# reglab/aquaculture

Hardware: AMD Instinct MI355X
Metric: 640px tiles/sec (whole node) YOLOv5m bf16 (higher is better)
Workload: dtype bf16

## Files before the change

aquaculture_amd/csrc/conv1x1_direct.hip:

```cpp
#include "conv_device.h"

using namespace aqdev;

namespace {

struct C1Params {
    const char* in;
    char* out;
    const char* w;
    const float* bias;
    const char* zero;
    int in_ld_b, out_ld_b;
    int npix, n_tiles, act;
    float out_inv_scale;
};

constexpr int kNW = 12;

template <int KS, int MBT, int MBW, int NBW> struct C1Geom {
    static constexpr int CIN = 32 * KS, COUT = 16 * MBT, CB = CIN / 8;
    static constexpr int MG = MBT / MBW;
    static constexpr int PG = kNW / MG;
    static constexpr int TP = PG * NBW * 16;
    static constexpr int SPP = CB + 2;
    static constexpr int PXB = SPP * 16;
    static constexpr int NQ = (TP * SPP + 63) / 64;
    static constexpr int XPB = NQ * 1024;
    static constexpr int LDS = 2 * XPB + COUT * 4;
    static constexpr int NST = NBW;
    static_assert(MBT % MBW == 0 && kNW % MG == 0 && LDS <= 160 * 1024, "shape");
};

__device__ __forceinline__ f32x4 c1_silu4(f32x4 v) {
    const f32x4 t = v * -1.44269504f;
    f32x4 d = {__builtin_amdgcn_exp2f(t[0]), __builtin_amdgcn_exp2f(t[1]), __builtin_amdgcn_exp2f(t[2]), __builtin_amdgcn_exp2f(t[3])};
    d = d + 1.0f;
    const f32x4 r = {__builtin_amdgcn_rcpf(d[0]), __builtin_amdgcn_rcpf(d[1]), __builtin_amdgcn_rcpf(d[2]), __builtin_amdgcn_rcpf(d[3])};
    return v * r;
}

template <int KS, int MBT, int MBW, int NBW, bool F8OUT = false>
__global__ __launch_bounds__(kNW * 64) void conv1x1_direct_kernel(const C1Params p) {
    using G = C1Geom<KS, MBT, MBW, NBW>;
    extern __shared__ __attribute__((aligned(16))) char smem[];
    float* s_b = (float*)(smem + 2 * G::XPB);

    const int tid = threadIdx.x, lane = tid & 63;
    const int wave = __builtin_amdgcn_readfirstlane(tid >> 6);
    static_assert(MBW == 2, "the paired-row layout below is written for two M blocks per wave");
    const int mb0 = (wave % G::MG) * MBW, pg = wave / G::MG;
    const int g = lane >> 4, l15 = lane & 15;
    const int cbase = mb0 * 16 + g * 8;

    bf16x8 wv[KS][MBW];
#pragma unroll
    for (int s = 0; s < KS; ++s)
#pragma unroll
        for (int m = 0; m < MBW; ++m) wv[s][m] = ((const bf16x8*)p.w)[((size_t)(mb0 + m) * KS + s) * 64 + lane];
    for (int i = tid; i < G::COUT; i += kNW * 64) s_b[i] = p.bias[i];

    auto issue_dma = [&](int tile, char* xb) {
        const long long n0 = (long long)tile * G::TP;
#pragma unroll 1
        for (int q = wave; q < G::NQ; q += kNW) {
            const int slot = q * 64 + lane;
            const int px = slot / G::SPP, part = slot - px * G::SPP;
            const bool valid = px < G::TP && part < G::CB && n0 + px < p.npix;
            const char* src = p.in + (n0 + px) * p.in_ld_b + part * 16;
            glds16(valid ? src : p.zero, xb + q * 1024);
        }
    };

    int tile = first_tile(gridDim.x, blockIdx.x);
    if (tile < p.n_tiles) issue_dma(tile, smem);
    int cur = 0;
    bool prev_full = false;
    for (; tile < p.n_tiles; tile += gridDim.x, cur ^= 1) {
        const long long n0 = (long long)tile * G::TP;
        const char* s_x = smem + cur * G::XPB;
        if (prev_full) wait_vmcnt<G::NST>(); else wait_vmcnt<0>();
        asm volatile("s_waitcnt lgkmcnt(0)" ::: "memory");
        __builtin_amdgcn_s_barrier();
        asm volatile("" ::: "memory");
// ... 27 lines not shown
                    q0[e] = __builtin_amdgcn_fmed3f(q0[e], -448.0f, 448.0f);
                    q1[e] = __builtin_amdgcn_fmed3f(q1[e], -448.0f, 448.0f);
                }
                int w0 = __builtin_amdgcn_cvt_pk_fp8_f32(q0[0], q0[1], 0, false);
                w0 = __builtin_amdgcn_cvt_pk_fp8_f32(q0[2], q0[3], w0, true);
                int w1 = __builtin_amdgcn_cvt_pk_fp8_f32(q1[0], q1[1], 0, false);
                w1 = __builtin_amdgcn_cvt_pk_fp8_f32(q1[2], q1[3], w1, true);
                if (n0 + px < p.npix) *(uint2*)(p.out + (n0 + px) * p.out_ld_b + cbase) = make_uint2((unsigned)w0, (unsigned)w1);
            } else if (n0 + px < p.npix)
                *(uint4*)(p.out + (n0 + px) * p.out_ld_b + cbase * 2) =
                    make_uint4(pack_bf16x2(v0[0], v0[1]), pack_bf16x2(v0[2], v0[3]), pack_bf16x2(v1[0], v1[1]), pack_bf16x2(v1[2], v1[3]));
        }
    }
}

template <int KS, int MBT, int MBW, int NBW, bool F8OUT = false>
int launch_c1(C1Params p, hipStream_t stream) {
    using G = C1Geom<KS, MBT, MBW, NBW>;
    auto fn = conv1x1_direct_kernel<KS, MBT, MBW, NBW, F8OUT>;
    int cus = 0;
    AQ_CHECK_HIP(aq_kernel_lds((const void*)fn, G::LDS));
    AQ_CHECK_HIP(aq_cus(&cus));
    p.n_tiles = (p.npix + G::TP - 1) / G::TP;
    long long grid = cus;
    if (grid > p.n_tiles) grid = p.n_tiles;
    hipLaunchKernelGGL(fn, dim3((unsigned)grid), dim3(kNW * 64), G::LDS, stream, p);
    AQ_CHECK_HIP(hipGetLastError());
    return AQ_OK;
}

}

extern "C" int aq_conv1x1_direct_supported(int cin, int cout) {
    return (cin == 96 && cout == 96) || (cin == 192 && cout == 192) || (cin == 384 && (cout == 192 || cout == 384));
// ... 30 lines not shown
               "conv1x1_direct: channel slices must be 8-aligned and inside their rows");
    C1Params p{};
    p.in = (const char*)in_dev + (size_t)in_choff * 2; p.in_ld_b = in_ld * 2;
    p.out = (char*)out_dev + (size_t)out_choff * 2; p.out_ld_b = out_ld * 2;
    p.w = (const char*)packed_w_dev; p.bias = bias_dev;
    p.npix = (int)npix; p.act = act;
    p.zero = aq_zero_page();
    AQ_REQUIRE(p.zero, "conv1x1_direct: zero page allocation failed");
    const hipStream_t st = (hipStream_t)stream;
    if (cin == 96) return launch_c1<3, 6, 2, 4>(p, st);
    if (cin == 192) return launch_c1<6, 12, 2, 4>(p, st);
    if (cout == 192) return launch_c1<12, 12, 2, 2>(p, st);
    return launch_c1<12, 24, 2, 4>(p, st);
}


extern "C" int aq_conv1x1_direct_f8out(const void* in_dev, int in_ld, int in_choff, void* out_dev, int out_pitch_bytes, int out_byte_off, int cin,
                                       int cout, const void* packed_w_dev, const float* bias_dev, long long npix, int act, float out_scale,
                                       void* stream) {
    AQ_REQUIRE(in_dev && out_dev && packed_w_dev && bias_dev, "conv1x1_direct_f8out: null pointer");
    AQ_REQUIRE((cin == 192 && cout == 192) || (cin == 384 && cout == 384), "conv1x1_direct_f8out: unsupported %d -> %d", cin, cout);
    AQ_REQUIRE(npix > 0 && sg::conv1x1_direct_fits(npix) && out_scale > 0.0f, "conv1x1_direct_f8out: bad pixel count or scale");
    AQ_REQUIRE(in_ld % 8 == 0 && in_choff % 8 == 0 && in_choff + cin <= in_ld && out_pitch_bytes % 8 == 0 && out_byte_off % 8 == 0 &&
                   out_byte_off + cout <= out_pitch_bytes, "conv1x1_direct_f8out: slices must be 8-byte aligned and inside their rows");
    C1Params p{};
    p.in = (const char*)in_dev + (size_t)in_choff * 2; p.in_ld_b = in_ld * 2;
    p.out = (char*)out_dev + out_byte_off; p.out_ld_b = out_pitch_bytes;
    p.w = (const char*)packed_w_dev; p.bias = bias_dev;
    p.npix = (int)npix; p.act = act; p.out_inv_scale = 1.0f / out_scale;
    p.zero = aq_zero_page();
// ... 6 lines not shown
```

aquaculture_amd/csrc/engine.cpp:

```cpp
#include "aq_common.h"
#include <unistd.h>
#include <string>

#include <cstdarg>
#include <cstdio>
#include <cstdlib>
#include <cstring>
#include <string>
#include <atomic>
#include <dlfcn.h>
#include <vector>

namespace {
thread_local char g_err[512] = "";
}

void aq_set_error(const char* fmt, ...) {
    va_list ap;
    va_start(ap, fmt);
    vsnprintf(g_err, sizeof(g_err), fmt, ap);
    va_end(ap);
}

extern "C" const char* aq_last_error(void) { return g_err; }
// ... 123 lines not shown
}

struct aq_engine {
    int device = 0;
    aq_model_desc desc{};
    std::vector<aq_tensor_desc> tensors;
    std::vector<aq_op_desc> ops;
    std::vector<PackedW> packed;
    std::vector<int> conv_cfg;
    int nms_agnostic = 0;
    unsigned long long nms_cls_lo = ~0ULL, nms_cls_hi = ~0ULL;
    struct Tuned { int B = 0, H = 0, W = 0; std::vector<int> cfg; };
    std::vector<Tuned> tuned;
    int tuned_cur = -1;
    bool tuning = false;
    void* zero_page = nullptr;
    int lay_B = 0, lay_H = 0, lay_W = 0;
    bool lay_aug = false;
    int run_H = 0, run_W = 0;
    std::vector<TensorPlace> place;
    size_t off_pred = 0, off_cand = 0, off_cand_rows = 0, off_cand_count = 0, off_cand_wide = 0, off_nms = 0, off_taps = 0, total_bytes = 0;
    int N = 0;
    aq_augment_pass aug[3] = {};
    std::vector<int> aug_family[3], aug_cfg[3];
    void* last_ws = nullptr;
    const uint8_t* last_tiles = nullptr;
    float* calib_amax = nullptr;
    std::vector<int> last_family, last_cfg;
    bool prof = false;
    int ring = 0;
// ... 305 lines not shown
}

bool c3tail_active(aq_engine* e, int oi, int last, int B) {
    if (!e->packed[oi].w_tail || oi + 1 >= last || e->calib_amax || e->tuning) return false;
    const int ci = oi + 1;
    const PackedW& pc = e->packed[ci];
    if (pc.direct_cfg != AQ_CONV_CFG_DIRECT1X1 || (pc.f8_consumer >= 0 && f8_pair_active(e, pc.f8_consumer, B))) return false;
    const aq_engine::Tuned* tt = tuned_for(e);
    const int cfg = e->conv_cfg[ci] >= 0 ? e->conv_cfg[ci] : tt ? tt->cfg[ci] : -1;
    if (cfg != AQ_CONV_CFG_DIRECT1X1) return false;
    const aq_op_desc& b = e->ops[oi];
    const aq_op_desc& c = e->ops[ci];
    const TensorPlace& pl = e->place[b.src.tensor];
    return aq_bottleneck_c3tail_supported(B, pl.h, pl.w, e->tensors[b.src.tensor].channels, e->tensors[c.src.tensor].channels,
                                          e->tensors[c.dst.tensor].channels) != 0;
}

struct AugRun {
    int pass;
    const aq_augment_pass* ps;
    int H0, W0;
    const aq_tap* ytab;
    const aq_tap* xtab;
};

int run_plan(aq_engine* e, const uint8_t* tiles, int B, int H, int W, void* ws, size_t ws_bytes,
             float* pred_out, aq_det* dets, int32_t* counts, float conf, float iou, int max_det, hipStream_t stream,
             int first = 0, int last = -1, const AugRun* ar = nullptr) {
    AQ_REQUIRE(e && tiles && ws, "infer: null pointer");
    const int n_ops = (int)e->ops.size();
// ... 21 lines not shown
    int32_t* cand_count = (int32_t*)((char*)ws + e->off_cand_count);
    float* cand_rows = (float*)((char*)ws + e->off_cand_rows);
    const char* use_sd = getenv("AQ_STEMDOWN");
    const bool stemdown = use_sd && *use_sd == '1' && prec == AQ_BF16 && n_ops > 2 && e->ops[0].kind == AQ_OP_STEM && e->ops[1].kind == AQ_OP_DOWNBLOCK &&
                          e->ops[0].dst.channels == 48 && e->ops[1].src.tensor == e->ops[0].dst.tensor && e->ops[1].src.ch_off == e->ops[0].dst.ch_off &&
                          aq_stemdown_supported(H, W) && ((uintptr_t)tiles & 3) == 0 && !scaled;
    const bool fuse_heads = dets != nullptr && heads_fused(e);
    bool heads_started = ar != nullptr;
    int heads_done = 0;
    for (int oi = 0; oi < first; ++oi)
        if (fuse_heads && e->ops[oi].kind == AQ_OP_CONV && e->ops[oi].level >= 0) {
            heads_started = true;
            ++heads_done;
        }
    int tail_conv = -1;
    for (int oi = first; oi < last; ++oi) {
        const aq_op_desc& op = e->ops[oi];
        if (ev) AQ_CHECK_HIP(hipEventRecord(ev[oi], stream));
        const bool mark = g_roctx.on();
        if (mark) {
            char name[96];
            snprintf(name, sizeof name, "aq op %02d kind %d: %d -> %d ch, k%d s%d%s", oi, op.kind, op.src.channels, op.dst.channels, op.k, op.stride,
                     op.level >= 0 ? " (detect head)" : "");
            g_roctx.push(name);
        }
        switch (op.kind) {
        case AQ_OP_PREPROCESS:
            if (scaled)
                rc = aq_preprocess_s2d_scaled(tiles, ar->H0, ar->W0, ar->ytab, ar->xtab, ar->ps->h, ar->ps->w, tptr(e, ws, tiles, op.dst.tensor), B, H, W,
                                              prec, stream);
            else
                rc = aq_preprocess_s2d(tiles, tptr(e, ws, tiles, op.dst.tensor), B, H, W, prec, stream);
            break;
        case AQ_OP_CONV:
            if (oi == tail_conv) {
                note_launch(e, oi, AQ_FAM_DIRECT1X1, AQ_CONV_CFG_DIRECT1X1);
                break;
            }
            if (ar && op.level >= 0 && !((ar->ps->level_mask >> op.level) & 1)) {
                note_launch(e, oi, AQ_FAM_NONE);
                break;
            }
            if (fuse_heads && op.level >= 0) {
                int32_t* wide = (int32_t*)((char*)ws + e->off_cand_wide);
                if (!heads_started) {
                    AQ_CHECK_HIP(hipMemsetAsync(wide, 0, sizeof(int32_t) * B * kCountStride, stream));
                    heads_started = true;
                }
                const TensorPlace& pl = e->place[op.src.tensor];
                int off = 0;
                for (int l = 0; l < op.level; ++l) off += e->desc.na * (H / (int)e->desc.stride[l]) * (W / (int)e->desc.stride[l]);
// ... 61 lines not shown
                                 e->packed[0].w, e->packed[0].bias, e->packed[oi].w, e->packed[oi].bias, B, H, W, stream);
                break;
            }
            rc = aq_downblock(tptr(e, ws, tiles, op.src.tensor), e->tensors[op.src.tensor].channels, op.src.ch_off,
                              tptr(e, ws, tiles, op.dst.tensor), e->tensors[op.dst.tensor].channels, op.dst.ch_off,
                              e->packed[oi].w, e->packed[oi].bias, B, pl.h, pl.w, stream);
            break;
        }
        case AQ_OP_SPPF_POOL: {
            const TensorPlace& pl = e->place[op.src.tensor];
            rc = aq_sppf_pool(tptr(e, ws, tiles, op.src.tensor), e->tensors[op.src.tensor].channels, op.src.ch_off,
                              op.src.channels, B, pl.h, pl.w, prec, stream);
            break;
        }
        case AQ_OP_UPSAMPLE2X: {
            const TensorPlace& pl = e->place[op.src.tensor];
            rc = aq_upsample2x(tptr(e, ws, tiles, op.src.tensor), e->tensors[op.src.tensor].channels, op.src.ch_off,
                               tptr(e, ws, tiles, op.dst.tensor), e->tensors[op.dst.tensor].channels, op.dst.ch_off,
                               op.src.channels, B, pl.h, pl.w, prec, stream);
            break;
        }
        case AQ_OP_DECODE: {
            if (fuse_heads) break;
            const float* heads[3];
            for (int l = 0; l < 3; ++l) heads[l] = (const float*)tptr(e, ws, tiles, e->desc.head_tensor[l]);
            float anchors[3 * 8 * 2];
            for (int l = 0; l < 3; ++l)
                for (int a = 0; a < e->desc.na; ++a) {
                    anchors[(l * e->desc.na + a) * 2] = e->desc.anchors_px[l][a][0];
                    anchors[(l * e->desc.na + a) * 2 + 1] = e->desc.anchors_px[l][a][1];
// ... 199 lines not shown
    if (x3) compute_desc.precision = AQ_FP32;
    d = &compute_desc;
    e->desc = *d;
    e->tensors.assign(d->tensors, d->tensors + d->n_tensors);
    e->ops.assign(d->ops, d->ops + d->n_ops);
    e->desc.tensors = e->tensors.data();
    e->desc.ops = e->ops.data();
    e->packed.resize(e->ops.size());
    e->conv_cfg.assign(e->ops.size(), -1);
    const int eb = aq_elem_bytes(d->precision);
    auto fail = [&](int rc) { aq_engine_destroy(e); return rc; };
    if (hipMalloc(&e->zero_page, 4096) != hipSuccess || hipMemset(e->zero_page, 0, 4096) != hipSuccess) {
        aq_set_error("engine_create: zero page allocation failed");
        return fail(AQ_ERR_NOMEM);
    }
    const char* use_tail = getenv("AQ_C3TAIL");
    for (size_t oi = 0; d->precision == AQ_BF16 && !(use_tail && *use_tail == '0') && oi + 1 < e->ops.size(); ++oi) {
        const aq_op_desc& b = e->ops[oi];
        const aq_op_desc& c = e->ops[oi + 1];
        if (b.kind != AQ_OP_BOTTLENECK || c.kind != AQ_OP_CONV || !b.weight || !b.bias || !c.weight || !c.bias) continue;
        if (b.src.channels != 48 || b.dst.channels != 48 || b.k != 3 || b.dst.tensor < 0 || b.dst.tensor >= d->n_tensors || b.dst.ch_off != 0 ||
            e->tensors[b.dst.tensor].channels != 96 || b.src.tensor == b.dst.tensor)
            continue;
        if (c.k != 1 || c.stride != 1 || c.act != 1 || c.res.tensor >= 0 || c.level >= 0 || c.src.tensor != b.dst.tensor || c.src.ch_off != 0 ||
            c.src.channels != 96 || c.dst.channels != 96 || c.dst.tensor < 0 || c.dst.tensor >= d->n_tensors || c.dst.tensor == c.src.tensor ||
            c.dst.tensor == b.src.tensor || c.dst.ch_off % 8 || e->tensors[c.dst.tensor].channels % 8 || e->tensors[c.dst.tensor].dtype != AQ_T_ACT)
            continue;
        bool read_later = false;
        for (size_t oj = oi + 2; oj < e->ops.size(); ++oj)
            for (const aq_slice* s : {&e->ops[oj].src, &e->ops[oj].res})
// ... 551 lines not shown
```

aquaculture_amd/csrc/size_guards.h:

```cpp
#pragma once

namespace sg {

typedef long long ll;

constexpr ll cdiv(ll a, ll b) { return (a + b - 1) / b; }

constexpr ll kStemTW = 64, kStemTH = 8;
constexpr ll kDownTW = 16, kDownblockTH = 8, kConv3x3s2TH = 4;
constexpr ll btl_tile_w(ll C) { return C == 16 ? 32 : 16; }
constexpr ll btl_tile_h(ll C) { return C == 96 ? 8 : 16; }

inline bool preprocess_fits(ll B, ll H, ll W) { return B * (H / 2) * (W / 2) < (1LL << 31); }
inline bool sppf_pool_fits(ll B, ll H, ll W, ll groups) { return B * H * W * groups < (1LL << 31); }
inline bool upsample2x_fits(ll B, ll H, ll W, ll groups) { return B * 4 * H * W * groups < (1LL << 31); }
inline bool upsample2x_rows_fit(ll B, ll H) { return B * H < 65536; }

inline bool tile_bytes_fit(ll B, ll H, ll W) { return B * H * W * 3 < (1LL << 40); }

inline bool stem_out_fits(ll B, ll Ho, ll Wo) {
    return B * Ho * Wo < (1LL << 31) && B * cdiv(Wo, kStemTW) * cdiv(Ho, kStemTH) < (1LL << 31);
}
inline bool stem_fits(ll B, ll H, ll W) { return B * H * W * 3 < (1LL << 32) && stem_out_fits(B, H / 2, W / 2); }

// ... 2 lines not shown
}
inline bool downblock_fits(ll B, ll H, ll W) { return down_fits(B, H, W, kDownblockTH); }
inline bool conv3x3s2_direct_fits(ll B, ll H, ll W) { return down_fits(B, H, W, kConv3x3s2TH); }

inline bool bottleneck_fits(ll C, ll B, ll H, ll W) {
    return B * H * W < (1LL << 31) && B * cdiv(W, btl_tile_w(C)) * cdiv(H, btl_tile_h(C)) < (1LL << 30);
}
inline bool btl_asm_tiles_fit(ll C, ll B, ll H, ll W, ll in_ld, ll out_ld) {
    const ll tx = cdiv(W, 16), tpi = tx * cdiv(H, btl_tile_h(C)), nt = tpi * B;
    return tx >= 2 && tpi >= 2 && nt < (1LL << 24) && nt * tpi < (1LL << 32) &&
           B * H * W * in_ld * 2 < (1LL << 30) && B * H * W * out_ld * 2 < (1LL << 31);
}
inline bool c3tail_cat_fits(ll B, ll H, ll W, ll cat_ld) { return B * H * W * cat_ld * 2 < (1LL << 31); }

inline bool conv1x1_direct_fits(ll npix) { return npix < (1LL << 31); }
inline bool conv1x1_asm_fits(ll npix, ll in_ld, ll out_ld) {
    return npix * in_ld * 2 < (1LL << 31) - (1LL << 22) && npix * out_ld * 2 < (1LL << 32) - (1LL << 22);
}

inline bool pl3x3_index_fits(ll B, ll H, ll W) { return B * (H + 1) * (W + 1) + W + 2 < (1LL << 23); }
inline bool pl3x3_offsets_fit(ll B, ll H, ll W, ll out_ld, ll res_ld) {
    return B * H * W * out_ld * 2 < (1LL << 31) && B * H * W * res_ld * 2 < (1LL << 31);
}
inline bool pl3x3s2_fits(ll B, ll H, ll W, ll in_ld, ll out_ld) {
    return pl3x3_index_fits(B, H / 2, W / 2) && B * (H / 2) * (W / 2) * out_ld * 2 < (1LL << 31) && B * H * W * in_ld * 2 < (1LL << 31) &&
           in_ld * 2 < (1LL << 24);
}
inline bool pl3x3_f8_offsets_fit(ll B, ll H, ll W, ll in_ld_bytes, ll out_ld, ll res_ld) {
    return pl3x3_offsets_fit(B, H, W, out_ld, res_ld) && B * H * W * in_ld_bytes < (1LL << 31) && in_ld_bytes < (1LL << 24);
}
// ... 36 lines not shown
```

aquaculture_amd/engine.py:

```python
from __future__ import annotations

import ctypes as C
import os
import re
from typing import Dict, List, Optional, Sequence, Tuple

import numpy as np
import torch

from . import spec as _spec
from .checkpoint import Checkpoint, pack_plan_weights

AQ_BF16, AQ_FP32, AQ_BF16_W8, AQ_F16X3 = 0, 1, 2, 3
PRECISIONS = {"bf16": AQ_BF16, "fp32": AQ_FP32, "fp8w": AQ_BF16, "f16x3": AQ_F16X3}
"""Compute precision of the single-op helpers.  fp8w = fp8 (OCP e4m3fn) weights with per-output-channel power-of-two scales, bf16
activations (quant.py): values bf16 holds exactly, so every bf16 kernel runs them as they are."""
ENGINE_PRECISIONS = {"bf16": AQ_BF16, "fp32": AQ_FP32, "fp8w": AQ_BF16_W8, "f16x3": AQ_F16X3, "fp8": AQ_BF16}
"""aq_model_desc.precision.  AQ_BF16_W8 computes as AQ_BF16; kernels with an fp8-weight stream (the planar 3x3) load the e4m3 codes."""
_DTYPE_CODE = {"act": 0, "f32": 1, "u8": 2}

LIB_PATH = os.path.join(os.path.dirname(os.path.abspath(__file__)), "csrc", "libaqengine.so")


class aq_tensor_desc(C.Structure):
# ... 17 lines not shown
                ("head_tensor", C.c_int32 * 3), ("input_tensor", C.c_int32),
                ("n_tensors", C.c_int32), ("n_ops", C.c_int32),
                ("tensors", C.POINTER(aq_tensor_desc)), ("ops", C.POINTER(aq_op_desc))]


class aq_det(C.Structure):
    _fields_ = [("x1", C.c_float), ("y1", C.c_float), ("x2", C.c_float), ("y2", C.c_float),
                ("conf", C.c_float), ("cls", C.c_float)]


EXPORTS = (
    "aq_last_error", "aq_version", "aq_engine_create", "aq_engine_destroy", "aq_engine_workspace_bytes", "aq_size_guard",
    "aq_engine_infer", "aq_engine_run_ops", "aq_engine_candidates", "aq_engine_forward_raw", "aq_engine_tensor_ptr", "aq_engine_profile",
    "aq_engine_op_times", "aq_engine_num_ops", "aq_engine_set_conv_config", "aq_engine_autotune", "aq_engine_set_tuned_table",
    "aq_engine_get_conv_config", "aq_conv_num_configs", "aq_debug_conv_stamp", "aq_debug_mfma_peak",
    "aq_conv_config_tiles", "aq_pack_conv_weights", "aq_pack_conv_weights_x3", "aq_conv2d", "aq_pack_stem_weights", "aq_stem_conv", "aq_pack_bottleneck_weights", "aq_bottleneck", "aq_bottleneck_asm_form", "aq_bottleneck_c3tail_supported", "aq_pack_bottleneck_c3tail_weights", "aq_bottleneck_c3tail", "aq_pack_downblock_weights", "aq_downblock", "aq_stemdown_supported", "aq_stemdown", "aq_conv1x1_direct_supported", "aq_pack_conv1x1_direct", "aq_conv1x1_direct", "aq_conv1x1_asm_supported", "aq_pack_conv1x1_asm", "aq_conv1x1_asm", "aq_nms_opts", "aq_engine_set_nms_options",
    "aq_conv3x3s2_direct_supported", "aq_pack_conv3x3s2_direct", "aq_conv3x3s2_direct",
    "aq_conv3x3_pl_supported", "aq_conv3x3_pl_asm_family", "aq_pack_conv3x3_pl", "aq_conv3x3_pl", "aq_conv3x3_pl_s2_supported", "aq_pack_conv3x3_pl_s2", "aq_conv3x3_pl_s2", "aq_jpeg_scratch_bytes", "aq_jpeg_idct_rgb", "aq_jpeg_idct_rgb_checked", "aq_f32_to_e4m3", "aq_conv1x1_direct_f8out", "aq_absmax_bf16", "aq_engine_calibrate_amax", "aq_engine_set_fp8_scales", "aq_engine_last_launch", "aq_conv3x3_pl_f8_supported", "aq_pack_conv3x3_pl_f8", "aq_conv3x3_pl_f8", "aq_conv3x3_pl_w8_supported", "aq_pack_conv3x3_pl_w8", "aq_conv3x3_pl_w8", "aq_head_decode_supported", "aq_pack_head_weights", "aq_head_decode", "aq_head_counts_gather", "aq_preprocess_s2d", "aq_sppf_pool",
    "aq_upsample2x", "aq_letterbox_u8", "aq_letterbox_tiles_u8", "aq_format_label_rows", "aq_detect_decode", "aq_nms_scratch_bytes", "aq_nms", "aq_jpeg_huffman_decode", "aq_write_label_files",
    "aq_crop_jpeg_coefs", "aq_crop_jpeg_bytes", "aq_write_crop_files",
    "aq_annotate_u8", "aq_image_jpeg_coefs", "aq_image_jpeg_bytes", "aq_write_image_files",
    "aq_blank_stats_scratch_bytes", "aq_blank_stats_u8",
    "aq_blank_geom_scratch_bytes", "aq_blank_components_u8", "aq_blank_ring_edges_u8",
    "aq_facility_scratch_bytes", "aq_facility_dbscan_f64",
    "aq_land_scratch_bytes", "aq_land_filter_f64",
    "aq_land_images_scratch_bytes", "aq_land_images_f64",
    "aq_eval_scratch_bytes", "aq_eval_member_conf_f64", "aq_box_match_f64",
    "aq_eval_subsets_scratch_bytes", "aq_eval_member_conf_subsets_f64", "aq_box_match_subsets_scratch_bytes", "aq_box_match_subsets_f64",
    "aq_model_error_match_f64", "aq_model_error_moments_f64",
    "aq_tonnage_simulate_f64", "aq_tonnage_reduce_f64", "aq_tonnage_ndtri_f64", "aq_tonnage_uniform_f64",
    "aq_depth_ranges_f64", "aq_depth_stats_f64",
# ... 99 lines not shown
    lib.aq_conv2d.argtypes = [vp, i32, i32, i32, vp, i32, i32, i32, vp, i32, i32, vp, vp,
                              i32, i32, i32, i32, i32, i32, i32, i32, i32, vp, vp]
    lib.aq_pack_stem_weights.argtypes = [C.POINTER(f32), i32, i32, vp, C.POINTER(sz), vp]
    lib.aq_stem_conv.argtypes = [vp, vp, i32, i32, i32, vp, vp, i32, i32, i32, i32, i32, vp]
    lib.aq_pack_bottleneck_weights.argtypes = [C.POINTER(f32), C.POINTER(f32), i32, vp, C.POINTER(sz), vp]
    lib.aq_bottleneck.argtypes = [vp, i32, i32, vp, i32, i32, i32, vp, vp, i32, i32, i32, i32, vp]
    lib.aq_bottleneck_asm_form.argtypes = [i32] * 6
    lib.aq_bottleneck_c3tail_supported.argtypes = [i32, i32, i32, i32, i32, i32]
    lib.aq_pack_bottleneck_c3tail_weights.argtypes = [C.POINTER(f32), C.POINTER(f32), C.POINTER(f32), vp, C.POINTER(sz), vp]
    lib.aq_bottleneck_c3tail.argtypes = [vp, i32, i32, vp, i32, i32, vp, i32, i32, vp, vp, i32, i32, i32, i32, vp]
    lib.aq_pack_downblock_weights.argtypes = [C.POINTER(f32), C.POINTER(f32), vp, C.POINTER(sz), vp]
    lib.aq_downblock.argtypes = [vp, i32, i32, vp, i32, i32, vp, vp, i32, i32, i32, vp]
    lib.aq_conv1x1_direct_supported.argtypes = [i32, i32]
    lib.aq_pack_conv1x1_direct.argtypes = [C.POINTER(f32), i32, i32, vp, C.POINTER(sz), vp]
    lib.aq_conv1x1_direct.argtypes = [vp, i32, i32, vp, i32, i32, i32, i32, vp, vp, C.c_longlong, i32, vp]
    lib.aq_nms_opts.argtypes = [vp, i32, i32, i32, i32, f32, f32, i32, vp, vp, i32, vp, vp, vp, i32, C.c_ulonglong, C.c_ulonglong, vp]
    lib.aq_engine_set_nms_options.argtypes = [vp, i32, C.c_ulonglong, C.c_ulonglong]
    lib.aq_conv1x1_asm_supported.argtypes = [i32, i32]
    lib.aq_pack_conv1x1_asm.argtypes = [C.POINTER(f32), i32, i32, vp, C.POINTER(sz), vp]
    lib.aq_conv1x1_asm.argtypes = [vp, i32, i32, vp, i32, i32, i32, i32, vp, vp, C.c_longlong, i32, vp]
    lib.aq_conv3x3s2_direct_supported.argtypes = [i32, i32]
    lib.aq_pack_conv3x3s2_direct.argtypes = [C.POINTER(f32), i32, i32, vp, C.POINTER(sz), vp]
    lib.aq_conv3x3s2_direct.argtypes = [vp, i32, i32, vp, i32, i32, i32, i32, vp, vp, i32, i32, i32, i32, vp]
    lib.aq_conv3x3_pl_supported.argtypes = [i32, i32]
    lib.aq_conv3x3_pl_asm_family.argtypes = [i32]
    lib.aq_pack_conv3x3_pl.argtypes = [C.POINTER(f32), i32, i32, vp, C.POINTER(sz), vp]
    lib.aq_conv3x3_pl.argtypes = [vp, C.c_longlong, C.c_longlong, i32, vp, i32, i32, i32, vp, i32, i32, vp, vp, i32, i32, i32, i32, vp]
    lib.aq_conv3x3_pl_w8.argtypes = lib.aq_conv3x3_pl.argtypes
    lib.aq_pack_conv3x3_pl_w8.argtypes = [C.POINTER(C.c_float), C.POINTER(C.c_float), i32, i32, vp, C.POINTER(C.c_size_t), vp, vp]
    lib.aq_conv3x3_pl_w8_supported.argtypes = [i32] * 5
# ... 1833 lines not shown
    w = np.ascontiguousarray(w_oihw.reshape(cout, cin).float().cpu().numpy())
    n = C.c_size_t()
    wp = w.ctypes.data_as(C.POINTER(C.c_float))
    _check(lib.aq_pack_conv1x1_direct(wp, cin, cout, None, C.byref(n), None))
    wbuf = torch.empty(n.value, dtype=torch.uint8, device=x.device)
    _check(lib.aq_pack_conv1x1_direct(wp, cin, cout, wbuf.data_ptr(), C.byref(n), _stream_ptr()))
    bbuf = bias.float().to(x.device).contiguous()
    if out is None:
        out = torch.empty(x.shape[:-1] + (cout,), dtype=torch.bfloat16, device=x.device)
    _check(lib.aq_conv1x1_direct(x.data_ptr(), ld, 0, out.data_ptr(), out.stride(-2), 0, cin, cout, wbuf.data_ptr(), bbuf.data_ptr(), npix, int(act),
                                 _stream_ptr()))
    torch.cuda.current_stream().synchronize()
    return out


def conv1x1_asm_nhwc(x: torch.Tensor, w_oihw: torch.Tensor, bias: torch.Tensor, out: Optional[torch.Tensor] = None) -> torch.Tensor:
    _require_gpu()
    lib = load_library()
    assert x.dtype == torch.bfloat16 and x.stride(-1) == 1
    cin, cout = x.shape[-1], w_oihw.shape[0]
    ld = x.stride(-2)
    npix = x.numel() // cin
    w = np.ascontiguousarray(w_oihw.reshape(cout, cin).float().cpu().numpy())
    n = C.c_size_t()
    wp = w.ctypes.data_as(C.POINTER(C.c_float))
    _check(lib.aq_pack_conv1x1_asm(wp, cin, cout, None, C.byref(n), None))
    wbuf = torch.empty(n.value, dtype=torch.uint8, device=x.device)
    _check(lib.aq_pack_conv1x1_asm(wp, cin, cout, wbuf.data_ptr(), C.byref(n), _stream_ptr()))
    bbuf = bias.float().to(x.device).contiguous()
    if out is None:
# ... 285 lines not shown
```

include/aq_engine.h:

```cpp
#ifndef AQ_ENGINE_H
#define AQ_ENGINE_H

#include <stddef.h>
#include <stdint.h>

#ifdef __cplusplus
extern "C" {
#endif

typedef enum aq_status {
    AQ_OK = 0,
    AQ_ERR_INVALID = -1,
    AQ_ERR_HIP = -2,
    AQ_ERR_NOMEM = -3,
    AQ_ERR_WORKSPACE = -4
} aq_status;

typedef enum aq_precision {
    AQ_BF16 = 0,
    AQ_FP32 = 1,
    AQ_BF16_W8 = 2,
    AQ_F16X3 = 3
} aq_precision;

// ... 138 lines not shown
                         void* stream);

int aq_pack_downblock_weights(const float* wa_host, const float* wb_host, void* packed_dev, size_t* bytes, void* stream);
int aq_downblock(const void* in_dev, int in_ld, int in_choff, void* out_dev, int out_ld, int out_choff,
                 const void* packed_w_dev, const float* bias_dev, int B, int H, int W, void* stream);
int aq_stemdown_supported(int Hi, int Wi);
int aq_stemdown(const uint8_t* tiles_dev, void* out_dev, int out_ld, int out_choff, const void* stem_w_dev, const float* stem_bias_dev,
                const void* packed_w_dev, const float* bias_dev, int B, int Hi, int Wi, void* stream);

#define AQ_CONV_CFG_DIRECT1X1 1000
#define AQ_CONV_CFG_ONE_TILE_PER_WG 4096
int aq_conv1x1_direct_supported(int cin, int cout);
int aq_pack_conv1x1_direct(const float* w_host, int cin, int cout, void* packed_dev, size_t* bytes, void* stream);
int aq_conv1x1_direct(const void* in_dev, int in_ld, int in_choff, void* out_dev, int out_ld, int out_choff, int cin, int cout,
                      const void* packed_w_dev, const float* bias_dev, long long npix, int act, void* stream);

#define AQ_CONV_CFG_ASM1X1 1004
int aq_conv1x1_asm_supported(int cin, int cout);
int aq_pack_conv1x1_asm(const float* w_host, int cin, int cout, void* packed_dev, size_t* bytes, void* stream);
int aq_conv1x1_asm(const void* in_dev, int in_ld, int in_choff, void* out_dev, int out_ld, int out_choff, int cin, int cout,
                   const void* packed_w_dev, const float* bias_dev, long long npix, int act, void* stream);

#define AQ_CONV_CFG_DIRECT3X3S2 1001
int aq_conv3x3s2_direct_supported(int cin, int cout);
int aq_pack_conv3x3s2_direct(const float* w_host, int cin, int cout, void* packed_dev, size_t* bytes, void* stream);
int aq_conv3x3s2_direct(const void* in_dev, int in_ld, int in_choff, void* out_dev, int out_ld, int out_choff, int cin, int cout,
                        const void* packed_w_dev, const float* bias_dev, int B, int H, int W, int act, void* stream);
#define AQ_CONV_CFG_PL3X3 1002
int aq_conv3x3_pl_supported(int cin, int cout);
int aq_conv3x3_pl_asm_family(int nb);
// ... 233 lines not shown
```

Baseline: 16930.

## Fold nearest 2x upsample into following 1x1 direct conv input gather

Adds an up2x variant of the direct 1x1 conv kernel. For channels belonging to the upsampled slice, it loads directly from the low-resolution tensor using a magic-number divide index map, instead of from the materialized upsampled concat buffer. The engine skips the standalone upsample op when the next op is an eligible 384->192 direct 1x1 conv whose upsampled slice has no other readers. This removes one kernel launch and the write and re-read of the upsampled tensor, at the cost of extra per-slot index arithmetic in the DMA issue loop and a scattered low-res read pattern.

```diff
diff --git a/aquaculture_amd/csrc/conv1x1_direct.hip b/aquaculture_amd/csrc/conv1x1_direct.hip
--- a/aquaculture_amd/csrc/conv1x1_direct.hip
+++ b/aquaculture_amd/csrc/conv1x1_direct.hip
@@ -1,4 +1,7 @@
 #include "conv_device.h"
+#include "upfold_index.h"
+
+#include <type_traits>
 
 using namespace aqdev;
 
@@ -13,6 +16,12 @@
     int in_ld_b, out_ld_b;
     int npix, n_tiles, act;
     float out_inv_scale;
+};
+
+struct C1UpParams : C1Params {
+    const char* up;
+    int up_ld_b, up_cb;
+    upfold::Map map;
 };
 
 constexpr int kNW = 12;
@@ -39,8 +48,8 @@
     return v * r;
 }
 
-template <int KS, int MBT, int MBW, int NBW, bool F8OUT = false>
-__global__ __launch_bounds__(kNW * 64) void conv1x1_direct_kernel(const C1Params p) {
+template <int KS, int MBT, int MBW, int NBW, bool F8OUT = false, bool UP = false>
+__global__ __launch_bounds__(kNW * 64) void conv1x1_direct_kernel(const std::conditional_t<UP, C1UpParams, C1Params> p) {
     using G = C1Geom<KS, MBT, MBW, NBW>;
     extern __shared__ __attribute__((aligned(16))) char smem[];
     float* s_b = (float*)(smem + 2 * G::XPB);
@@ -67,6 +76,10 @@
             const int px = slot / G::SPP, part = slot - px * G::SPP;
             const bool valid = px < G::TP && part < G::CB && n0 + px < p.npix;
             const char* src = p.in + (n0 + px) * p.in_ld_b + part * 16;
+            if constexpr (UP) {
+                const char* lo = p.up + (long long)upfold::up2x_src_pixel(p.map, (unsigned)(n0 + px)) * p.up_ld_b + part * 16;
+                src = part < p.up_cb ? lo : src;
+            }
             glds16(valid ? src : p.zero, xb + q * 1024);
         }
     };
@@ -124,10 +137,10 @@
     }
 }
 
-template <int KS, int MBT, int MBW, int NBW, bool F8OUT = false>
-int launch_c1(C1Params p, hipStream_t stream) {
+template <int KS, int MBT, int MBW, int NBW, bool F8OUT = false, bool UP = false>
+int launch_c1(std::conditional_t<UP, C1UpParams, C1Params> p, hipStream_t stream) {
     using G = C1Geom<KS, MBT, MBW, NBW>;
-    auto fn = conv1x1_direct_kernel<KS, MBT, MBW, NBW, F8OUT>;
+    auto fn = conv1x1_direct_kernel<KS, MBT, MBW, NBW, F8OUT, UP>;
     int cus = 0;
     AQ_CHECK_HIP(aq_kernel_lds((const void*)fn, G::LDS));
     AQ_CHECK_HIP(aq_cus(&cus));
@@ -188,6 +201,37 @@
     return launch_c1<12, 24, 2, 4>(p, st);
 }
 
+extern "C" int aq_conv1x1_direct_up2x_supported(int cin, int cout, int c_up, int B, int Hl, int Wl, int up_ld) {
+    return cin == 384 && cout == 192 && c_up == 192 && sg::conv1x1_up2x_fits(B, Hl, Wl, up_ld) && sg::conv1x1_direct_fits((sg::ll)B * 4 * Hl * Wl);
+}
+
+extern "C" long long aq_up2x_src_pixel(long long n, int B, int Hl, int Wl) {
+    if (!sg::conv1x1_up2x_fits(B, Hl, Wl, 1) || n < 0 || n >= (long long)B * 4 * Hl * Wl) return -1;
+    return upfold::up2x_src_pixel(upfold::up2x_map((unsigned)Hl, (unsigned)Wl), (unsigned)n);
+}
+
+extern "C" int aq_conv1x1_direct_up2x(const void* up_dev, int up_ld, int up_choff, int c_up, int B, int Hl, int Wl, const void* in_dev, int in_ld,
+                                      int in_choff, void* out_dev, int out_ld, int out_choff, int cin, int cout, const void* packed_w_dev,
+                                      const float* bias_dev, int act, void* stream) {
+    AQ_REQUIRE(up_dev && in_dev && out_dev && packed_w_dev && bias_dev, "conv1x1_direct_up2x: null pointer");
+    AQ_REQUIRE(B > 0 && Hl > 0 && Wl > 0 && up_ld > 0, "conv1x1_direct_up2x: empty input");
+    AQ_REQUIRE(aq_conv1x1_direct_up2x_supported(cin, cout, c_up, B, Hl, Wl, up_ld), "conv1x1_direct_up2x: unsupported %d (%d upsampled) -> %d at %d x %d x %d",
+               cin, c_up, cout, B, Hl, Wl);
+    AQ_REQUIRE(in_ld % 8 == 0 && out_ld % 8 == 0 && in_choff % 8 == 0 && out_choff % 8 == 0 && in_choff + cin <= in_ld && out_choff + cout <= out_ld &&
+                   up_ld % 8 == 0 && up_choff % 8 == 0 && up_choff >= 0 && up_choff + c_up <= up_ld,
+               "conv1x1_direct_up2x: channel slices must be 8-aligned and inside their rows");
+    C1UpParams p{};
+    p.in = (const char*)in_dev + (size_t)in_choff * 2; p.in_ld_b = in_ld * 2;
+    p.out = (char*)out_dev + (size_t)out_choff * 2; p.out_ld_b = out_ld * 2;
+    p.w = (const char*)packed_w_dev; p.bias = bias_dev;
+    p.npix = B * 4 * Hl * Wl; p.act = act;
+    p.up = (const char*)up_dev + (size_t)up_choff * 2; p.up_ld_b = up_ld * 2; p.up_cb = c_up / 8;
+    p.map = upfold::up2x_map((unsigned)Hl, (unsigned)Wl);
+    p.zero = aq_zero_page();
+    AQ_REQUIRE(p.zero, "conv1x1_direct_up2x: zero page allocation failed");
+    return launch_c1<12, 12, 2, 2, false, true>(p, (hipStream_t)stream);
+}
+
 
 extern "C" int aq_conv1x1_direct_f8out(const void* in_dev, int in_ld, int in_choff, void* out_dev, int out_pitch_bytes, int out_byte_off, int cin,
                                        int cout, const void* packed_w_dev, const float* bias_dev, long long npix, int act, float out_scale,
diff --git a/aquaculture_amd/csrc/engine.cpp b/aquaculture_amd/csrc/engine.cpp
--- a/aquaculture_amd/csrc/engine.cpp
+++ b/aquaculture_amd/csrc/engine.cpp
@@ -161,6 +161,7 @@
     std::vector<Tuned> tuned;
     int tuned_cur = -1;
     bool tuning = false;
+    bool upfold = true;
     void* zero_page = nullptr;
     int lay_B = 0, lay_H = 0, lay_W = 0;
     bool lay_aug = false;
@@ -496,6 +497,29 @@
     const TensorPlace& pl = e->place[b.src.tensor];
     return aq_bottleneck_c3tail_supported(B, pl.h, pl.w, e->tensors[b.src.tensor].channels, e->tensors[c.src.tensor].channels,
                                           e->tensors[c.dst.tensor].channels) != 0;
+}
+
+bool upfold_active(aq_engine* e, int oi, int last, int B, bool aug) {
+    if (!e->upfold || aug || oi + 1 >= last || e->calib_amax || e->tuning || e->desc.precision != AQ_BF16) return false;
+    const int ci = oi + 1;
+    const aq_op_desc& u = e->ops[oi];
+    const aq_op_desc& c = e->ops[ci];
+    if (c.kind != AQ_OP_CONV || c.k != 1 || c.stride != 1 || c.res.tensor >= 0 || c.level >= 0) return false;
+    if (c.src.tensor != u.dst.tensor || c.src.ch_off != u.dst.ch_off || u.src.channels != u.dst.channels || u.src.tensor == u.dst.tensor ||
+        c.dst.tensor == c.src.tensor || c.dst.tensor == u.src.tensor || e->tensors[c.dst.tensor].dtype != AQ_T_ACT)
+        return false;
+    for (int oj = 0; oj < (int)e->ops.size(); ++oj)
+        for (const aq_slice* s : {&e->ops[oj].src, &e->ops[oj].res})
+            if (oj != ci && s->tensor == u.dst.tensor && s->ch_off < u.dst.ch_off + u.dst.channels && u.dst.ch_off < s->ch_off + s->channels) return false;
+    const PackedW& pc = e->packed[ci];
+    if (pc.direct_cfg != AQ_CONV_CFG_DIRECT1X1 || (pc.f8_consumer >= 0 && f8_pair_active(e, pc.f8_consumer, B))) return false;
+    const aq_engine::Tuned* tt = tuned_for(e);
+    const int cfg = e->conv_cfg[ci] >= 0 ? e->conv_cfg[ci] : tt ? tt->cfg[ci] : -1;
+    if (cfg != AQ_CONV_CFG_DIRECT1X1) return false;
+    const TensorPlace& lo = e->place[u.src.tensor];
+    const TensorPlace& hi = e->place[c.src.tensor];
+    return hi.h == 2 * lo.h && hi.w == 2 * lo.w &&
+           aq_conv1x1_direct_up2x_supported(c.src.channels, c.dst.channels, u.dst.channels, B, lo.h, lo.w, e->tensors[u.src.tensor].channels) != 0;
 }
 
 struct AugRun {
@@ -547,6 +571,7 @@
             ++heads_done;
         }
     int tail_conv = -1;
+    int fold_conv = -1;
     for (int oi = first; oi < last; ++oi) {
         const aq_op_desc& op = e->ops[oi];
         if (ev) AQ_CHECK_HIP(hipEventRecord(ev[oi], stream));
@@ -568,6 +593,16 @@
         case AQ_OP_CONV:
             if (oi == tail_conv) {
                 note_launch(e, oi, AQ_FAM_DIRECT1X1, AQ_CONV_CFG_DIRECT1X1);
+                break;
+            }
+            if (oi == fold_conv) {
+                const aq_op_desc& u = e->ops[oi - 1];
+                const TensorPlace& lo = e->place[u.src.tensor];
+                note_launch(e, oi, AQ_FAM_DIRECT1X1, AQ_CONV_CFG_DIRECT1X1);
+                rc = aq_conv1x1_direct_up2x(tptr(e, ws, tiles, u.src.tensor), e->tensors[u.src.tensor].channels, u.src.ch_off, u.dst.channels, B, lo.h, lo.w,
+                                            tptr(e, ws, tiles, op.src.tensor), e->tensors[op.src.tensor].channels, op.src.ch_off,
+                                            tptr(e, ws, tiles, op.dst.tensor), e->tensors[op.dst.tensor].channels, op.dst.ch_off,
+                                            op.src.channels, op.dst.channels, e->packed[oi].w_direct, e->packed[oi].bias, op.act, stream);
                 break;
             }
             if (ar && op.level >= 0 && !((ar->ps->level_mask >> op.level) & 1)) {
@@ -659,6 +694,10 @@
             break;
         }
         case AQ_OP_UPSAMPLE2X: {
+            if (upfold_active(e, oi, last, B, ar != nullptr)) {
+                fold_conv = oi + 1;
+                break;
+            }
             const TensorPlace& pl = e->place[op.src.tensor];
             rc = aq_upsample2x(tptr(e, ws, tiles, op.src.tensor), e->tensors[op.src.tensor].channels, op.src.ch_off,
                                tptr(e, ws, tiles, op.dst.tensor), e->tensors[op.dst.tensor].channels, op.dst.ch_off,
@@ -888,6 +927,8 @@
         aq_set_error("engine_create: zero page allocation failed");
         return fail(AQ_ERR_NOMEM);
     }
+    const char* use_fold = getenv("AQ_UPFOLD");
+    e->upfold = !(use_fold && *use_fold == '0');
     const char* use_tail = getenv("AQ_C3TAIL");
     for (size_t oi = 0; d->precision == AQ_BF16 && !(use_tail && *use_tail == '0') && oi + 1 < e->ops.size(); ++oi) {
         const aq_op_desc& b = e->ops[oi];
diff --git a/aquaculture_amd/csrc/size_guards.h b/aquaculture_amd/csrc/size_guards.h
--- a/aquaculture_amd/csrc/size_guards.h
+++ b/aquaculture_amd/csrc/size_guards.h
@@ -40,6 +40,9 @@
 inline bool c3tail_cat_fits(ll B, ll H, ll W, ll cat_ld) { return B * H * W * cat_ld * 2 < (1LL << 31); }
 
 inline bool conv1x1_direct_fits(ll npix) { return npix < (1LL << 31); }
+inline bool conv1x1_up2x_fits(ll B, ll Hl, ll Wl, ll up_ld) {
+    return B >= 1 && Hl >= 1 && Wl >= 1 && up_ld >= 1 && B * 4 * Hl * Wl < (1LL << 31) && B * Hl * Wl * up_ld * 2 < (1LL << 40);
+}
 inline bool conv1x1_asm_fits(ll npix, ll in_ld, ll out_ld) {
     return npix * in_ld * 2 < (1LL << 31) - (1LL << 22) && npix * out_ld * 2 < (1LL << 32) - (1LL << 22);
 }
diff --git a/aquaculture_amd/csrc/upfold_index.h b/aquaculture_amd/csrc/upfold_index.h
--- /dev/null
+++ b/aquaculture_amd/csrc/upfold_index.h
@@ -0,0 +1,38 @@
+#pragma once
+
+#if defined(__HIPCC__)
+#define AQ_UPFOLD_HD __host__ __device__
+#else
+#define AQ_UPFOLD_HD
+#endif
+
+namespace upfold {
+
+struct Magic { unsigned m, s; };
+
+inline Magic up2x_magic(unsigned d) {
+    unsigned t = 1;
+    while ((1ULL << t) < d) ++t;
+    const unsigned long long p = 1ULL << (31 + t);
+    return Magic{(unsigned)((p + d - 1) / d), t - 1};
+}
+
+AQ_UPFOLD_HD inline unsigned up2x_div(unsigned n, Magic g) { return (unsigned)(((unsigned long long)n * g.m) >> 32) >> g.s; }
+
+struct Map {
+    unsigned hw, w, hl, wl;
+    Magic by_hw, by_w;
+};
+
+inline Map up2x_map(unsigned Hl, unsigned Wl) {
+    const unsigned H = 2 * Hl, W = 2 * Wl;
+    return Map{H * W, W, Hl, Wl, up2x_magic(H * W), up2x_magic(W)};
+}
+
+AQ_UPFOLD_HD inline unsigned up2x_src_pixel(const Map& g, unsigned n) {
+    const unsigned b = up2x_div(n, g.by_hw), r = n - b * g.hw;
+    const unsigned y = up2x_div(r, g.by_w), x = r - y * g.w;
+    return (b * g.hl + (y >> 1)) * g.wl + (x >> 1);
+}
+
+}
diff --git a/aquaculture_amd/engine.py b/aquaculture_amd/engine.py
--- a/aquaculture_amd/engine.py
+++ b/aquaculture_amd/engine.py
@@ -55,7 +55,7 @@
     "aq_engine_infer", "aq_engine_run_ops", "aq_engine_candidates", "aq_engine_forward_raw", "aq_engine_tensor_ptr", "aq_engine_profile",
     "aq_engine_op_times", "aq_engine_num_ops", "aq_engine_set_conv_config", "aq_engine_autotune", "aq_engine_set_tuned_table",
     "aq_engine_get_conv_config", "aq_conv_num_configs", "aq_debug_conv_stamp", "aq_debug_mfma_peak",
-    "aq_conv_config_tiles", "aq_pack_conv_weights", "aq_pack_conv_weights_x3", "aq_conv2d", "aq_pack_stem_weights", "aq_stem_conv", "aq_pack_bottleneck_weights", "aq_bottleneck", "aq_bottleneck_asm_form", "aq_bottleneck_c3tail_supported", "aq_pack_bottleneck_c3tail_weights", "aq_bottleneck_c3tail", "aq_pack_downblock_weights", "aq_downblock", "aq_stemdown_supported", "aq_stemdown", "aq_conv1x1_direct_supported", "aq_pack_conv1x1_direct", "aq_conv1x1_direct", "aq_conv1x1_asm_supported", "aq_pack_conv1x1_asm", "aq_conv1x1_asm", "aq_nms_opts", "aq_engine_set_nms_options",
+    "aq_conv_config_tiles", "aq_pack_conv_weights", "aq_pack_conv_weights_x3", "aq_conv2d", "aq_pack_stem_weights", "aq_stem_conv", "aq_pack_bottleneck_weights", "aq_bottleneck", "aq_bottleneck_asm_form", "aq_bottleneck_c3tail_supported", "aq_pack_bottleneck_c3tail_weights", "aq_bottleneck_c3tail", "aq_pack_downblock_weights", "aq_downblock", "aq_stemdown_supported", "aq_stemdown", "aq_conv1x1_direct_supported", "aq_pack_conv1x1_direct", "aq_conv1x1_direct", "aq_conv1x1_direct_up2x_supported", "aq_up2x_src_pixel", "aq_conv1x1_direct_up2x", "aq_conv1x1_asm_supported", "aq_pack_conv1x1_asm", "aq_conv1x1_asm", "aq_nms_opts", "aq_engine_set_nms_options",
     "aq_conv3x3s2_direct_supported", "aq_pack_conv3x3s2_direct", "aq_conv3x3s2_direct",
     "aq_conv3x3_pl_supported", "aq_conv3x3_pl_asm_family", "aq_pack_conv3x3_pl", "aq_conv3x3_pl", "aq_conv3x3_pl_s2_supported", "aq_pack_conv3x3_pl_s2", "aq_conv3x3_pl_s2", "aq_jpeg_scratch_bytes", "aq_jpeg_idct_rgb", "aq_jpeg_idct_rgb_checked", "aq_f32_to_e4m3", "aq_conv1x1_direct_f8out", "aq_absmax_bf16", "aq_engine_calibrate_amax", "aq_engine_set_fp8_scales", "aq_engine_last_launch", "aq_conv3x3_pl_f8_supported", "aq_pack_conv3x3_pl_f8", "aq_conv3x3_pl_f8", "aq_conv3x3_pl_w8_supported", "aq_pack_conv3x3_pl_w8", "aq_conv3x3_pl_w8", "aq_head_decode_supported", "aq_pack_head_weights", "aq_head_decode", "aq_head_counts_gather", "aq_preprocess_s2d", "aq_sppf_pool",
     "aq_upsample2x", "aq_letterbox_u8", "aq_letterbox_tiles_u8", "aq_format_label_rows", "aq_detect_decode", "aq_nms_scratch_bytes", "aq_nms", "aq_jpeg_huffman_decode", "aq_write_label_files",
@@ -185,6 +185,10 @@
     lib.aq_conv1x1_direct_supported.argtypes = [i32, i32]
     lib.aq_pack_conv1x1_direct.argtypes = [C.POINTER(f32), i32, i32, vp, C.POINTER(sz), vp]
     lib.aq_conv1x1_direct.argtypes = [vp, i32, i32, vp, i32, i32, i32, i32, vp, vp, C.c_longlong, i32, vp]
+    lib.aq_conv1x1_direct_up2x_supported.argtypes = [i32, i32, i32, i32, i32, i32, i32]
+    lib.aq_up2x_src_pixel.argtypes = [C.c_longlong, i32, i32, i32]
+    lib.aq_up2x_src_pixel.restype = C.c_longlong
+    lib.aq_conv1x1_direct_up2x.argtypes = [vp, i32, i32, i32, i32, i32, i32, vp, i32, i32, vp, i32, i32, i32, i32, vp, vp, i32, vp]
     lib.aq_nms_opts.argtypes = [vp, i32, i32, i32, i32, f32, f32, i32, vp, vp, i32, vp, vp, vp, i32, C.c_ulonglong, C.c_ulonglong, vp]
     lib.aq_engine_set_nms_options.argtypes = [vp, i32, C.c_ulonglong, C.c_ulonglong]
     lib.aq_conv1x1_asm_supported.argtypes = [i32, i32]
@@ -2048,6 +2052,38 @@
     return out
 
 
+def pack_conv1x1_direct(w_oihw: torch.Tensor, bias: torch.Tensor, device) -> Tuple[torch.Tensor, torch.Tensor]:
+    lib = load_library()
+    cout, cin = w_oihw.shape[:2]
+    w = np.ascontiguousarray(w_oihw.reshape(cout, cin).float().cpu().numpy())
+    n = C.c_size_t()
+    wp = w.ctypes.data_as(C.POINTER(C.c_float))
+    _check(lib.aq_pack_conv1x1_direct(wp, cin, cout, None, C.byref(n), None))
+    wbuf = torch.empty(n.value, dtype=torch.uint8, device=device)
+    _check(lib.aq_pack_conv1x1_direct(wp, cin, cout, wbuf.data_ptr(), C.byref(n), _stream_ptr()))
+    return wbuf, bias.float().to(device).contiguous()
+
+
+def conv1x1_direct_up2x_nhwc(up: torch.Tensor, x: torch.Tensor, packed: Tuple[torch.Tensor, torch.Tensor], cout: int, act: bool = True,
+                             out: Optional[torch.Tensor] = None, sync: bool = True) -> torch.Tensor:
+    _require_gpu()
+    lib = load_library()
+    assert up.dtype == torch.bfloat16 and x.dtype == torch.bfloat16 and up.stride(3) == 1 and x.stride(3) == 1
+    B, Hl, Wl, c_up = up.shape
+    assert tuple(x.shape[:3]) == (B, 2 * Hl, 2 * Wl)
+    for t in (up, x):
+        assert t.stride(1) == t.shape[2] * t.stride(2) and t.stride(0) == t.shape[1] * t.stride(1)
+    cin = x.shape[3]
+    if out is None:
+        out = torch.empty((B, 2 * Hl, 2 * Wl, cout), dtype=torch.bfloat16, device=x.device)
+    assert out.stride(3) == 1 and out.stride(1) == out.shape[2] * out.stride(2) and out.stride(0) == out.shape[1] * out.stride(1)
+    _check(lib.aq_conv1x1_direct_up2x(up.data_ptr(), up.stride(2), 0, c_up, B, Hl, Wl, x.data_ptr(), x.stride(2), 0, out.data_ptr(), out.stride(2), 0,
+                                      cin, cout, packed[0].data_ptr(), packed[1].data_ptr(), int(act), _stream_ptr()))
+    if sync:
+        torch.cuda.current_stream().synchronize()
+    return out
+
+
 def conv1x1_asm_nhwc(x: torch.Tensor, w_oihw: torch.Tensor, bias: torch.Tensor, out: Optional[torch.Tensor] = None) -> torch.Tensor:
     _require_gpu()
     lib = load_library()
diff --git a/include/aq_engine.h b/include/aq_engine.h
--- a/include/aq_engine.h
+++ b/include/aq_engine.h
@@ -176,6 +176,11 @@
 int aq_pack_conv1x1_direct(const float* w_host, int cin, int cout, void* packed_dev, size_t* bytes, void* stream);
 int aq_conv1x1_direct(const void* in_dev, int in_ld, int in_choff, void* out_dev, int out_ld, int out_choff, int cin, int cout,
                       const void* packed_w_dev, const float* bias_dev, long long npix, int act, void* stream);
+int aq_conv1x1_direct_up2x_supported(int cin, int cout, int c_up, int B, int Hl, int Wl, int up_ld);
+long long aq_up2x_src_pixel(long long n, int B, int Hl, int Wl);
+int aq_conv1x1_direct_up2x(const void* up_dev, int up_ld, int up_choff, int c_up, int B, int Hl, int Wl, const void* in_dev, int in_ld,
+                           int in_choff, void* out_dev, int out_ld, int out_choff, int cin, int cout, const void* packed_w_dev,
+                           const float* bias_dev, int act, void* stream);
 
 #define AQ_CONV_CFG_ASM1X1 1004
 int aq_conv1x1_asm_supported(int cin, int cout);
```

Result: no change. 17090 (median of 6 runs) (+1.0%).
